# getzlab/rnaseqc

Hardware: AMD Instinct MI355X
Metric: reads/sec whole-node (100 M-read synthetic BAM, GENCODE GTF) at 1/2/4/8 GPU -- `value`: the hot path over the records resident in HBM (the bench contract's definition of value); `whole_node.value`: the same job from the BAM file to the reports (CLI `Average Reads/Sec` window), checked against `value (higher is better)
Workload: dtype i32/u64 counters, f64 exon fractions

## Files before the change

### rnaseqc_amd/csrc/rsqc_k1.h

```cpp
#pragma once

namespace rsqc {

#if defined(__HIP_DEVICE_COMPILE__)
#define K1E_LANDED(x) asm volatile("" : "+v"(x))
#ifdef K1E_PIN_ARGS
#define K1E_PIN(x) asm volatile("" : "+s"(x))
#else
#define K1E_PIN(x) (void)(x)
#endif
#else
#define K1E_LANDED(x) (void)(x)
#define K1E_PIN(x) (void)(x)
#endif

struct K1Args { DevAnnotation a; DevParams p; DevBatch b; DevAccum acc; };
#if defined(__HIPCC__)
__device__ __forceinline__ const K1Args *k1e_lazy_args() {
#if defined(__HIP_DEVICE_COMPILE__)
    const K1Args *q = (const K1Args *)__builtin_amdgcn_kernarg_segment_ptr();
    asm volatile("" : "+s"(q));
    return q;
#else
    return nullptr;
#endif
}
#else
static const K1Args *g_k1e_args = nullptr;
static unsigned long long g_k1e_coarse_hits = 0;
static unsigned long long g_k1e_ucache_hits = 0;
static unsigned long long g_k1e_uniform_calls = 0;
static unsigned long long g_k1e_uniform2_calls = 0;
static inline const K1Args *k1e_lazy_args() { return g_k1e_args; }
#endif

#ifndef K1E_NT
#define K1E_NT 0
#endif
template <class T> __device__ __forceinline__ T k1e_ld32_stream(const T *base, uint32_t idx) {
#if defined(__HIP_DEVICE_COMPILE__)
    if (K1E_NT & 1) {
        typedef uint32_t u32x4 __attribute__((ext_vector_type(4)));
        static_assert(sizeof(T) == 16, "16-byte streams");
        const u32x4 v = __builtin_nontemporal_load(reinterpret_cast<const u32x4 *>(reinterpret_cast<const char *>(base) + (uint32_t)(idx * 16u)));
        T r; __builtin_memcpy(&r, &v, 16); return r;
    }
#endif
    return ld32(base, idx);
}
struct alignas(4) Cig4 { uint32_t v[4]; };
__device__ __forceinline__ void k1e_load_cigar8(const uint32_t *cigar, uint32_t off, uint32_t (&c)[8]) {
    const char *const at = reinterpret_cast<const char *>(cigar) + (uint32_t)(off * 4u);
#if defined(__HIP_DEVICE_COMPILE__)
    if (K1E_NT & 1) {
        typedef uint32_t u32x4a __attribute__((ext_vector_type(4), aligned(4)));
        const u32x4a l4 = __builtin_nontemporal_load(reinterpret_cast<const u32x4a *>(at)), h4 = __builtin_nontemporal_load(reinterpret_cast<const u32x4a *>(at + 16));
        c[0] = l4.x; c[1] = l4.y; c[2] = l4.z; c[3] = l4.w; c[4] = h4.x; c[5] = h4.y; c[6] = h4.z; c[7] = h4.w;
        return;
    }
#endif
    const Cig4 lo = *reinterpret_cast<const Cig4 *>(at), hi = *reinterpret_cast<const Cig4 *>(at + 16);
#pragma unroll
    for (int k = 0; k < 4; ++k) { c[k] = lo.v[k]; c[4 + k] = hi.v[k]; }
}

#if defined(K1E_STOP_AT) && defined(__HIP_DEVICE_COMPILE__)
template <class T> __device__ __forceinline__ int k1e_keep_v(T x) { asm volatile("" :: "v"(x)); return 0; }
template <class T> __device__ __forceinline__ int k1e_keep_s(T x) { asm volatile("" :: "s"(x)); return 0; }
template <class... T> __device__ __forceinline__ void k1e_sink_v(T... x) { const int d[] = {k1e_keep_v(x)...}; (void)d; }
template <class... T> __device__ __forceinline__ void k1e_sink_s(T... x) { const int d[] = {k1e_keep_s(x)...}; (void)d; }
#define K1E_STOP(n, V, S) if (K1E_STOP_AT == (n)) { k1e_sink_v V; k1e_sink_s S; break; }
#else
#define K1E_STOP(n, V, S)
#endif
#if defined(K1E_STAGE_MARKS)
#define K1E_AMARK(sec)
#else
#define K1E_AMARK(sec) RSQC_MARK(sec)
#endif
constexpr int K1E_WAVES = RSQC_K1_THREADS / 64;
#ifndef K1E_PIECE_RECORDS
#define K1E_PIECE_RECORDS 256
#endif
constexpr uint64_t K1E_PIECE = K1E_PIECE_RECORDS;
#ifndef K1E_QCAP_N
#define K1E_QCAP_N 128
#endif
constexpr int K1E_QCAP = K1E_QCAP_N;
#ifndef K1E_ESLOTS_N
#define K1E_ESLOTS_N 256
#endif
#ifndef K1E_GSLOTS_N
#define K1E_GSLOTS_N 128
#endif
constexpr int K1E_ESLOTS = K1E_ESLOTS_N, K1E_GSLOTS = K1E_GSLOTS_N;
constexpr uint32_t K1E_HQ = 1u << 16;
#ifndef K1E_ABL
#define K1E_ABL 0
#endif
#ifndef K1E_WALK_SKIP
#define K1E_WALK_SKIP 1
#endif
#ifndef K1E_EXON_RUNSUM
#define K1E_EXON_RUNSUM 1
#endif

struct K1eTables {
    unsigned long long cnt[8];
    uint32_t cnt32[64];
    double eval[K1E_ESLOTS];
    uint32_t ekey[K1E_ESLOTS];
    unsigned long long gval[K1E_GSLOTS];
    uint32_t gkey[K1E_GSLOTS];
    uint32_t rl[3];
    uint32_t pairs;
    uint32_t frags;
    uint32_t piece;
    uint32_t defer;
    alignas(16) uint32_t ucache[K1E_WAVES][12];
    int32_t bedc[K1E_WAVES][4];
    static __device__ __forceinline__ constexpr int sum_slot(int c) {
        return c == RSQC_C_END1_MISMATCHES ? 0 : c == RSQC_C_END1_BASES ? 1 : c == RSQC_C_END2_MISMATCHES ? 2 : c == RSQC_C_END2_BASES ? 3 :
               c == RSQC_C_MISMATCHED_BASES ? 4 : c == RSQC_C_TOTAL_BASES ? 5 : c == RSQC_C_ALIGNMENT_BLOCKS ? 6 : 7;
    }
    __device__ __forceinline__ void init(uint32_t pairs0) {
        if (threadIdx.x < 8) cnt[threadIdx.x] = 0ull;
        if (threadIdx.x < 64) cnt32[threadIdx.x] = 0u;
        for (int c = threadIdx.x; c < K1E_ESLOTS; c += blockDim.x) { ekey[c] = 0xFFFFFFFFu; eval[c] = 0.0; }
        for (int c = threadIdx.x; c < K1E_GSLOTS; c += blockDim.x) { gkey[c] = 0xFFFFFFFFu; gval[c] = 0ull; }
        if (threadIdx.x == 0) { rl[0] = 0u; rl[1] = 0xFFFFFFFFu; rl[2] = 0u; pairs = pairs0; piece = 0u; frags = 0u; defer = 0u; }
        if (threadIdx.x < K1E_WAVES) { ucache[threadIdx.x][8] = 1u; ucache[threadIdx.x][9] = 0u; bedc[threadIdx.x][0] = -1; }
    }
    __device__ __forceinline__ void exon_add(uint32_t eid, double frac) {
        const uint32_t slot = eid & (K1E_ESLOTS - 1);
        const uint32_t old = atomicCAS(&ekey[slot], 0xFFFFFFFFu, eid);
        if (old == 0xFFFFFFFFu || old == eid) atomicAdd(&eval[slot], frac);
        else atomicAdd(&k1e_lazy_args()->acc.exon_acc[eid], frac);
    }
    __device__ __forceinline__ void gene_add(uint32_t g, uint32_t n, uint32_t nd) {
        const uint32_t slot = g & (K1E_GSLOTS - 1);
        const uint32_t old = atomicCAS(&gkey[slot], 0xFFFFFFFFu, g);
        if (old == 0xFFFFFFFFu || old == g) atomicAdd(&gval[slot], (unsigned long long)n | ((unsigned long long)nd << 32));
        else {
            const DevAccum &acc = k1e_lazy_args()->acc;
            atomicAdd(&acc.gene_reads[g], (unsigned long long)n); if (nd) atomicAdd(&acc.gene_unique[g], (unsigned long long)nd);
        }
    }
    __device__ __forceinline__ void flush(unsigned long long n_records) {
        const DevAccum &acc = k1e_lazy_args()->acc;
        for (int c = threadIdx.x; c < RSQC_N_COUNTERS; c += blockDim.x) {
            unsigned long long v = cnt[sum_slot(c)] + (unsigned long long)cnt32[c];
            if (c == RSQC_C_TOTAL_ALIGNMENTS) v += n_records;
            if (c == RSQC_C_MAPPED_UNIQUE_READS) v += (unsigned long long)cnt32[RSQC_C_MAPPED_READS] - cnt32[RSQC_C_MAPPED_DUPLICATE_READS];
            if (c == RSQC_C_UNIQUE_FRAGMENTS) v += (unsigned long long)cnt32[RSQC_C_END1_MAPPED_READS] - cnt32[RSQC_C_DUPLICATE_PAIRS];
            if (c == RSQC_C_LOW_QUALITY_READS) v += (unsigned long long)cnt32[RSQC_C_READS_USED] - cnt32[RSQC_C_HIGH_QUALITY_READS];
            if (v) atomicAdd(&acc.counters[c], v);
        }
        for (int c = threadIdx.x; c < K1E_ESLOTS; c += blockDim.x)
            if (ekey[c] != 0xFFFFFFFFu) atomicAdd(&acc.exon_acc[ekey[c]], eval[c]);
        for (int c = threadIdx.x; c < K1E_GSLOTS; c += blockDim.x)
            if (gkey[c] != 0xFFFFFFFFu) {
                const unsigned long long v = gval[c];
                atomicAdd(&acc.gene_reads[gkey[c]], v & 0xFFFFFFFFull);
                if (v >> 32) atomicAdd(&acc.gene_unique[gkey[c]], v >> 32);
            }
    }
};

struct K1eQueue1 { uint32_t bs[K1E_QCAP], lf[K1E_QCAP], idx[K1E_QCAP];
#ifdef K1E_COARSE
                   uint32_t cz[K1E_QCAP];
#endif
};
struct K1eQueue2 { uint32_t bs0[K1E_QCAP], len0[K1E_QCAP], bs1[K1E_QCAP], len1[K1E_QCAP], idx[K1E_QCAP], flhq[K1E_QCAP]; };
#ifndef K1E_Q3CAP_N
#define K1E_Q3CAP_N 84
#endif
constexpr int K1E_Q3CAP = K1E_Q3CAP_N;
static_assert(K1E_Q3CAP >= 64 && K1E_Q3CAP <= 128, "the three-block ring holds at least one full call");
struct K1eQueue3 { uint32_t bs0[K1E_Q3CAP], bs1[K1E_Q3CAP], bs2[K1E_Q3CAP], lens01[K1E_Q3CAP], lf2[K1E_Q3CAP], idx[K1E_Q3CAP]; };
__device__ __forceinline__ uint32_t k1e_wrap3(uint32_t s) { return s >= (uint32_t)K1E_Q3CAP ? s - (uint32_t)K1E_Q3CAP : s; }
struct K1eShared {
    K1eTables T;
    K1eQueue1 q1[K1E_WAVES];
    K1eQueue2 q2[K1E_WAVES];
    K1eQueue3 q3[K1E_WAVES];
#ifdef K1E_LDS_PAD
    char pad[K1E_LDS_PAD];
#endif
};

#if defined(__HIP_DEVICE_COMPILE__)
#define K1E_GLOBAL(T, p) ((__attribute__((address_space(1))) T *)(p))
#else
#define K1E_GLOBAL(T, p) (p)
#endif
struct K1ePairDst { uint64_t pairs; uint32_t cap; };
#ifndef K1E_LAZYPAIR
#define K1E_LAZYPAIR 1
#endif
__device__ __forceinline__ K1ePairDst k1e_pair_dst() {
    K1ePairDst d;
#if defined(__HIP_DEVICE_COMPILE__)
    const void *q = __builtin_amdgcn_kernarg_segment_ptr();
    asm volatile("s_load_dwordx2 %0, %2, %3\n\ts_load_dword %1, %2, %4\n\ts_waitcnt lgkmcnt(0)"
                 : "=&s"(d.pairs), "=&s"(d.cap)
                 : "s"(q), "n"(offsetof(K1Args, acc) + offsetof(DevAccum, pairs)), "n"(offsetof(K1Args, acc) + offsetof(DevAccum, pair_chunk_cap)));
#else
    const DevAccum &a = k1e_lazy_args()->acc;
    d.pairs = (uint64_t)(uintptr_t)a.pairs; d.cap = a.pair_chunk_cap;
#endif
    return d;
}
#ifndef K1E_CONSTMASK
#define K1E_CONSTMASK 1
#endif
__device__ __forceinline__ bool k1e_first_lane() { return K1E_CONSTMASK ? WaveSink::lane(LaneMask{1ull}) : lane_id() == 0; }
template <int N> __device__ __forceinline__ bool k1e_lane_below() { static_assert(N > 0 && N < 64, "lanes"); return K1E_CONSTMASK ? WaveSink::lane(LaneMask{(1ull << N) - 1ull}) : lane_id() < N; }

template <bool LANE_CHUNK = false>
__device__ __forceinline__ void k1e_emit_pairs(K1eTables &T, uint64_t m, uint32_t g, uint64_t qhash, uint32_t qh2, const K1ePairDst &pd, uint32_t chunk) {
    if (LANE_CHUNK) {
        if (WaveSink::lane(LaneMask{m})) {
            const uint32_t slot = atomicAdd(&k1e_lazy_args()->acc.pair_chunk_count[chunk], 1u);
            if (slot < pd.cap) K1E_GLOBAL(PairRec, (PairRec *)(uintptr_t)pd.pairs)[(size_t)chunk * pd.cap + slot] = PairRec{g, qh2, qhash};
            else atomicExch(k1e_lazy_args()->acc.error, RSQC_ERR_CAPACITY);
        }
        return;
    }
    const int lead = __ffsll((unsigned long long)m) - 1;
    uint32_t base = 0;
    if (lane_id() == lead) base = atomicAdd(&T.pairs, (uint32_t)__popcll(m));
    base = lane_value(base, lead);
    if (WaveSink::lane(LaneMask{m})) {
        const uint32_t slot = base + mask_rank(m);
        const size_t chunk_at = (size_t)chunk * pd.cap;
        if (slot < pd.cap) {
#if defined(__HIP_DEVICE_COMPILE__)
            if (K1E_NT & 2) {
                typedef uint32_t u32x4 __attribute__((ext_vector_type(4)));
                const u32x4 v = {g, qh2, (uint32_t)qhash, (uint32_t)(qhash >> 32)};
                __builtin_nontemporal_store(v, reinterpret_cast<u32x4 *>(K1E_GLOBAL(PairRec, (PairRec *)(uintptr_t)pd.pairs) + (chunk_at + slot)));
            } else
#endif
            K1E_GLOBAL(PairRec, (PairRec *)(uintptr_t)pd.pairs)[chunk_at + slot] = PairRec{g, qh2, qhash};
        } else atomicExch(k1e_lazy_args()->acc.error, RSQC_ERR_CAPACITY);
    }
}

template <int NB, bool LANE_CHUNK = false>
__device__ __forceinline__ void k1e_commit(uint32_t *cov_diff, K1eTables &T, const EiOut &eo, const uint32_t (&len)[NB], uint32_t fl,
                                           uint64_t qhash, uint32_t qh2, const K1ePairDst &held, uint32_t chunk) {
    typedef WaveSink WS;
    const K1ePairDst pd = K1E_LAZYPAIR ? k1e_pair_dst() : held;
    const uint64_t notdup = WS::prim((fl & RSQC_FDUP) == 0).m;
    double inv_aligned = 1.0;
    uint32_t aligned_of = 0; (void)aligned_of;
    if (NB > 1) {
        uint32_t aligned = 0;
#pragma unroll
        for (int b = 0; b < NB; ++b) aligned += len[b];
        inv_aligned = 1.0 / (double)(aligned ? aligned : 1u);
        aligned_of = aligned;
    }
#pragma unroll
    for (int k = 0; k < 2 * NB; ++k) {
        const uint64_t has = WS::prim(((eo.cmask >> k) & 1u) != 0).m;
        if (has == 0ull) continue;
        const uint32_t ln = len[k >> 1];
        const uint64_t hvm = has & WS::prim(ln > 0).m;
        const bool hv = WS::lane(LaneMask{hvm});
        if (NB == 1) {
            const RunLite r = make_run_lite(hvm, eo.eid[k]);
            if (r.head && !(K1E_ABL & 2)) T.exon_add(eo.eid[k], (double)r.count);
            if (k == 0) {
                const uint64_t nd = hvm & notdup;
                if (r.head && !(K1E_ABL & 2)) T.gene_add(eo.hit[0], r.count, run_popcount(nd, r.count));
            }
        } else if (!(K1E_ABL & 2)) {
#if K1E_EXON_RUNSUM
            const uint64_t cont = run_cont_mask(hvm, eo.eid[k]);
            if (cont == 0ull) { if (hv) T.exon_add(eo.eid[k], (double)ln * inv_aligned); }
            else {
                const uint32_t al = aligned_of;
                const uint64_t mixed_len = cont & WS::prim(lane_below(al) != al).m;
                if (mixed_len != 0ull) { if (hv) T.exon_add(eo.eid[k], (double)ln * inv_aligned); }
                else {
                    const uint32_t sc = wave_inclusive_scan_u32_dpp(hv ? ln : 0u);
                    const uint32_t cnt_run = run_length_at(cont);
                    const uint32_t at_end = lane_gather(sc, (uint32_t)lane_id() + cnt_run - 1u);
                    const bool head = WS::lane(LaneMask{hvm & ~cont});
                    if (head) T.exon_add(eo.eid[k], (double)(at_end - (sc - ln)) * inv_aligned);
                }
            }
#else
            if (hv) T.exon_add(eo.eid[k], (double)ln * inv_aligned);
#endif
        }
        const uint32_t base = hv ? eo.cidx[k] : 0u;
        if (!(K1E_ABL & 4)) {
            cov_add_merged(cov_diff, hvm, base, 1u);
            cov_add_merged(cov_diff, hvm, base + ln, 0xFFFFFFFFu);
        }
    }
#pragma unroll
    for (int k = 0; k < FAST_SET; ++k) {
        const uint64_t m = WS::prim(eo.n_hit > k).m;
        if (m == 0ull) break;
        const uint32_t g = eo.hit[k];
        if (!(K1E_ABL & 8)) k1e_emit_pairs<LANE_CHUNK>(T, m, g, qhash, qh2, pd, chunk);
        if (NB > 1 || k > 0) {
            const RunLite r = make_run_lite(m, g);
            const uint64_t nd = m & notdup;
            if (r.head && !(K1E_ABL & 2)) T.gene_add(g, r.count, run_popcount(nd, r.count));
        }
    }
}

constexpr uint64_t K1E_OVF_LONG = 1ull << 63;
constexpr uint32_t K1E_OVF_STAGE = 1024;
struct K1eStageCtl {
    uint32_t n;
    uint32_t end;
    __device__ __forceinline__ void init() { n = 0u; end = K1E_OVF_STAGE; }
    __device__ __forceinline__ uint32_t staged() const { return n < end ? n : end; }
};
__device__ __forceinline__ void k1e_overflow(bool over, uint64_t index, unsigned long long *stage = nullptr, K1eStageCtl *ctl = nullptr) {
    const uint64_t m = WaveSink::prim(over).m;
    if (m == 0ull) return;
    const int lead = __ffsll((unsigned long long)m) - 1;
    const uint32_t n = (uint32_t)__popcll(m);
    uint32_t base = 0;
    bool staged = false;
    if (stage) {
        if (lane_id() == lead) base = atomicAdd(&ctl->n, n);
        base = lane_value(base, lead);
        staged = base <= K1E_OVF_STAGE - n;
        if (staged && over) stage[base + mask_rank(m)] = index;
        if (!staged && lane_id() == lead) atomicMin(&ctl->end, base);
    }
    if (!staged) {
        const DevAccum &acc = k1e_lazy_args()->acc;
        if (lane_id() == lead) base = atomicAdd(acc.ovf_count, n);
        base = lane_value(base, lead);
        if (over) {
            const uint32_t slot = base + mask_rank(m);
            if (slot < acc.ovf_cap) acc.ovf_index[slot] = index;
            else atomicExch(acc.error, RSQC_ERR_CAPACITY);
        }
    }
}
__device__ __forceinline__ void k1e_stage_flush(const DevAccum &acc, const unsigned long long *stage, const K1eStageCtl *ctl, uint32_t *piece) {
    const uint32_t n_st = ctl->staged();
    if (n_st != 0u) {
        if (threadIdx.x == 0) *piece = atomicAdd(acc.ovf_count, n_st);
        __syncthreads();
        const uint32_t at = *piece;
        for (uint32_t j = threadIdx.x; j < n_st; j += blockDim.x) {
            if (at + j < acc.ovf_cap) acc.ovf_index[at + j] = stage[j];
            else atomicExch(acc.error, RSQC_ERR_CAPACITY);
        }
    }
}

#ifndef K1E_UNIFORM1
#define K1E_UNIFORM1 1
#endif
// ... 59 lines not shown
    if (p.stranded != RSQC_STRAND_UNKNOWN || ci.rk_words == 0u) return false;
    uint32_t *const uc = T.ucache[wave]; (void)uc;
    EiEntry S;
    bool cached = false;
#if K1E_UCACHE
    {
        const int32_t lo = (int32_t)__builtin_amdgcn_readfirstlane((int)uc[8]), hi = (int32_t)__builtin_amdgcn_readfirstlane((int)uc[9]);
        cached = (WS::prim(bs < lo || (int32_t)(bs + (int32_t)len) >= hi).m & onm) == 0ull;
        if (cached) {
            const uint4 e0 = *reinterpret_cast<const uint4 *>(uc), e1 = *reinterpret_cast<const uint4 *>(uc + 4);
#define K1E_U(x) ((uint32_t)__builtin_amdgcn_readfirstlane((int)(x)))
            S = EiEntry{(int32_t)K1E_U(e0.x), K1E_U(e0.y), K1E_U(e0.z), K1E_U(e0.w), K1E_U(e1.x), K1E_U(e1.y), K1E_U(e1.z), K1E_U(e1.w)};
#undef K1E_U
#if defined(RSQC_WAVE_EMU)
            if (lane_id() == 0) ++g_k1e_ucache_hits;
#endif
        }
    }
#endif
    if (!cached) {
        const K1eInterval iv = k1e_interval_of(a, ci, (int32_t)lane_value((uint32_t)bs, 0));
        S = iv.S;
        if (S.mask & EIM_DEEP) return false;
        const int32_t lo = S.pos, hi = iv.next_pos > S.pos ? iv.next_pos : 0x7FFFFFFF;
        if ((WS::prim(bs < lo || (int32_t)(bs + (int32_t)len) >= hi).m & onm) != 0ull) return false;
#if K1E_UCACHE
        if (k1e_first_lane()) {
            *reinterpret_cast<uint4 *>(uc) = make_uint4((uint32_t)S.pos, S.mask, S.eidA, S.eidB);
            *reinterpret_cast<uint4 *>(uc + 4) = make_uint4(S.gfA, S.cdA, S.gfB, S.cdB);
            *reinterpret_cast<uint2 *>(uc + 8) = make_uint2((uint32_t)lo, (uint32_t)hi);
        }
        k1e_wave_lds_visible();
#endif
    }
#if defined(RSQC_WAVE_EMU)
    if (lane_id() == 0) ++g_k1e_uniform_calls;
#endif
    const bool cA = S.eidA != EI_NONE, cB = S.eidB != EI_NONE, c1 = cA && cB;
    const uint32_t g0 = S.gfA & ROW_GENE_MASK, g1 = S.gfB & ROW_GENE_MASK;
    const uint32_t gX = cA ? g0 : g1, gfX = cA ? S.gfA : S.gfB;
    const bool va = cA || cB, vb = c1 && g1 != gX;
    const bool globin = (va && ((gfX >> ROW_FLAG_SHIFT) & ROWF_GLOBIN) != 0) || (vb && ((S.gfB >> ROW_FLAG_SHIFT) & ROWF_GLOBIN) != 0);
    const uint64_t hqm = WS::prim((flhq & K1E_HQ) != 0).m & onm, dupm = WS::prim((flhq & RSQC_FDUP) != 0).m;
    const uint32_t n_on = (uint32_t)__popcll(onm), n_hq = (uint32_t)__popcll(hqm);
    if (!globin) {
        RSQC_COUNT(cnt, RSQC_C_NON_GLOBIN_READS, LaneMask{onm}); RSQC_COUNT(cnt, RSQC_C_NON_GLOBIN_DUPLICATE_READS, LaneMask{onm & dupm});
    }
    k1e_uniform_class_counts(p, ei_class_flags(S.mask, RSQC_STRAND_UNKNOWN), va, flhq, onm, n_on, n_hq, cnt);
    if (!va || hqm == 0ull) return true;
    const uint64_t hvm = hqm & WS::prim(len > 0).m;
    if (hvm == 0ull) return true;
    const K1ePairDst pd = K1E_LAZYPAIR ? k1e_pair_dst() : held;
    const uint32_t n0 = (uint32_t)__popcll(hvm), nd0 = (uint32_t)__popcll(hvm & ~dupm);
    const bool first = k1e_first_lane();
    if (!(K1E_ABL & 2)) {
        if (first) { T.exon_add(cA ? S.eidA : S.eidB, (double)n0); T.gene_add(gX, n0, nd0); }
        if (first && c1) T.exon_add(S.eidB, (double)n0);
        if (first && vb) T.gene_add(g1, n0, nd0);
    }
    if (!(K1E_ABL & 4)) {
        const uint32_t base = (cA ? S.cdA : S.cdB) + (uint32_t)bs;
        cov_add_merged(cov_diff, hvm, base, 1u); cov_add_merged(cov_diff, hvm, base + len, 0xFFFFFFFFu);
        if (c1) { const uint32_t b1 = S.cdB + (uint32_t)bs; cov_add_merged(cov_diff, hvm, b1, 1u); cov_add_merged(cov_diff, hvm, b1 + len, 0xFFFFFFFFu); }
    }
    if (!(K1E_ABL & 8)) {
        k1e_emit_pairs(T, hvm, gX, qhash, qh2, pd, blockIdx.x);
        if (vb) k1e_emit_pairs(T, hvm, g1, qhash, qh2, pd, blockIdx.x);
    }
    return true;
}

#ifndef K1E_UNIFORM2
#define K1E_UNIFORM2 0
#endif
struct K1eInterval2 { EiEntry S[2]; int32_t next_pos[2]; uint32_t next_mask[2]; };
__device__ __forceinline__ K1eInterval2 k1e_intervals_of(const DevAnnotation &a, const ContigInfo &ci, int32_t x0, int32_t x1) {
    const int32_t top = (int32_t)(ci.rk_words << 6) - 1;
    const int32_t xc0 = x0 < 0 ? 0 : (x0 > top ? top : x0), xc1 = x1 < 0 ? 0 : (x1 > top ? top : x1);
    const uint32_t word0 = ci.rk_base + ((uint32_t)xc0 >> 6), word1 = ci.rk_base + ((uint32_t)xc1 >> 6);
    K1eInterval2 r;
#if defined(__HIP_DEVICE_COMPILE__)
    typedef uint32_t u32x4 __attribute__((ext_vector_type(4)));
    typedef uint32_t u32x16 __attribute__((ext_vector_type(16)));
    u32x4 w0, w1;
    asm volatile("s_load_dwordx4 %0, %2, %3\n\ts_load_dwordx4 %1, %2, %4\n\ts_waitcnt lgkmcnt(0)"
                 : "=&s"(w0), "=&s"(w1) : "s"(a.ei_rank), "s"(word0 * 16u), "s"(word1 * 16u));
    const uint64_t t0 = (((uint64_t)w0.y << 32) | (uint64_t)w0.x) << (63u - ((uint32_t)xc0 & 63u));
    const uint64_t t1 = (((uint64_t)w1.y << 32) | (uint64_t)w1.x) << (63u - ((uint32_t)xc1 & 63u));
    const uint32_t j0 = w0.z + (uint32_t)__popcll(t0) - 1u, j1 = w1.z + (uint32_t)__popcll(t1) - 1u;
    u32x16 e0, e1;
    asm volatile("s_load_dwordx16 %0, %2, %3\n\ts_load_dwordx16 %1, %2, %4\n\ts_waitcnt lgkmcnt(0)"
                 : "=&s"(e0), "=&s"(e1) : "s"(a.ei), "s"(j0 * 32u), "s"(j1 * 32u));
    r.S[0] = EiEntry{(int32_t)e0.s0, e0.s1, e0.s2, e0.s3, e0.s4, e0.s5, e0.s6, e0.s7}; r.next_pos[0] = (int32_t)e0.s8; r.next_mask[0] = e0.s9;
    r.S[1] = EiEntry{(int32_t)e1.s0, e1.s1, e1.s2, e1.s3, e1.s4, e1.s5, e1.s6, e1.s7}; r.next_pos[1] = (int32_t)e1.s8; r.next_mask[1] = e1.s9;
#else
    const int32_t xc[2] = {xc0, xc1}; const uint32_t word[2] = {word0, word1};
    for (int b = 0; b < 2; ++b) {
        const EiRank w = a.ei_rank[word[b]];
        const uint64_t t = (((uint64_t)w.hi << 32) | (uint64_t)w.lo) << (63u - ((uint32_t)xc[b] & 63u));
        const uint32_t j = w.rank + (uint32_t)__builtin_popcountll(t) - 1u;
        r.S[b] = a.ei[j]; r.next_pos[b] = a.ei[j + 1].pos; r.next_mask[b] = a.ei[j + 1].mask;
    }
#endif
    return r;
}
__device__ __forceinline__ bool k1e_uniform2(const DevAnnotation &a, const DevParams &p, uint32_t *cov_diff, const ContigInfo &ci, K1eTables &T,
                                             const int32_t (&bs)[2], const uint32_t (&len)[2], uint32_t flhq, uint64_t qhash, uint32_t qh2,
                                             uint64_t onm, WaveSink &cnt, const K1ePairDst &held) {
    typedef WaveSink WS;
    if (p.stranded != RSQC_STRAND_UNKNOWN || ci.rk_words == 0u) return false;
    const K1eInterval2 iv = k1e_intervals_of(a, ci, (int32_t)lane_value((uint32_t)bs[0], 0), (int32_t)lane_value((uint32_t)bs[1], 0));
    if ((iv.S[0].mask | iv.S[1].mask) & EIM_DEEP) return false;
    uint32_t mask = 0;
#pragma unroll
    for (int b = 0; b < 2; ++b) {
        const int32_t lo = iv.S[b].pos, hi = iv.next_pos[b] > iv.S[b].pos ? iv.next_pos[b] : 0x7FFFFFFF;
        const int32_t be = bs[b] + (int32_t)len[b];
        if ((WS::prim(bs[b] < lo || bs[b] >= hi || be > hi).m & onm) != 0ull) return false;
        const uint64_t touch = WS::prim(be == hi).m & onm;
        if (touch != 0ull && touch != onm) return false;
        mask |= iv.S[b].mask | (touch != 0ull ? iv.next_mask[b] & ~EIM_DEEP : 0u);
    }
#if defined(RSQC_WAVE_EMU)
    if (lane_id() == 0) ++g_k1e_uniform2_calls;
#endif
    uint32_t eid[4], cd[4], con = 0, ma = 0, mb = 0, la = 0, lb = 0;
    bool va = false, vb = false, ga = false, gb = false;
#pragma unroll
    for (int b = 0; b < 2; ++b) {
        const EiEntry &S = iv.S[b];
        const bool cA = S.eidA != EI_NONE, cB = S.eidB != EI_NONE, c0 = cA || cB, c1 = cA && cB;
        const uint32_t g0 = S.gfA & ROW_GENE_MASK, g1 = S.gfB & ROW_GENE_MASK;
        const uint32_t gX = cA ? g0 : g1, gfX = cA ? S.gfA : S.gfB;
        eid[2 * b] = cA ? S.eidA : S.eidB; cd[2 * b] = cA ? S.cdA : S.cdB; eid[2 * b + 1] = S.eidB; cd[2 * b + 1] = S.cdB;
        con |= (c0 ? 1u : 0u) << (2 * b) | (c1 ? 1u : 0u) << (2 * b + 1);
        if (b == 0) {
            la = gX; va = c0; ga = c0 && ((gfX >> ROW_FLAG_SHIFT) & ROWF_GLOBIN) != 0;
            lb = g1; vb = c1 && g1 != gX; gb = vb && ((S.gfB >> ROW_FLAG_SHIFT) & ROWF_GLOBIN) != 0;
            ma = (c0 ? 1u : 0u) | ((c1 && g1 == gX) ? 2u : 0u); mb = vb ? 2u : 0u;
        } else {
            const bool a_in = (c0 && la == gX) || (c1 && la == g1), b_in = (c0 && lb == gX) || (c1 && lb == g1);
            va = va && a_in; vb = vb && b_in;
            ma |= ((c0 && la == gX) ? 1u : 0u) << 2 | ((c1 && la == g1) ? 1u : 0u) << 3;
            mb |= ((c0 && lb == gX) ? 1u : 0u) << 2 | ((c1 && lb == g1) ? 1u : 0u) << 3;
        }
    }
    ga = ga && va; gb = gb && vb;
    const bool any_gene = va || vb;
    const uint64_t hqm = WS::prim((flhq & K1E_HQ) != 0).m & onm, dupm = WS::prim((flhq & RSQC_FDUP) != 0).m;
    const uint32_t n_on = (uint32_t)__popcll(onm), n_hq = (uint32_t)__popcll(hqm);
    if (!(ga || gb)) {
        RSQC_COUNT(cnt, RSQC_C_NON_GLOBIN_READS, LaneMask{onm}); RSQC_COUNT(cnt, RSQC_C_NON_GLOBIN_DUPLICATE_READS, LaneMask{onm & dupm});
    }
    k1e_uniform_class_counts(p, ei_class_flags(mask, RSQC_STRAND_UNKNOWN), any_gene, flhq, onm, n_on, n_hq, cnt);
    if (!any_gene || hqm == 0ull) return true;
    const uint32_t cmask = con & ((va ? ma : 0u) | (vb ? mb : 0u));
    const K1ePairDst pd = K1E_LAZYPAIR ? k1e_pair_dst() : held;
    const uint32_t aligned = len[0] + len[1];
    const bool first = k1e_first_lane();
#pragma unroll
    for (int b = 0; b < 2; ++b) {
        const uint32_t bits = (cmask >> (2 * b)) & 3u;
        if (bits == 0u) continue;
        const uint32_t ln = len[b];
        const uint64_t hvm = hqm & WS::prim(ln > 0).m;
        if (hvm == 0ull) continue;
        const bool hv = WS::lane(LaneMask{hvm});
        if (!(K1E_ABL & 2)) {
            const uint32_t al0 = lane_value(aligned, __ffsll((unsigned long long)hvm) - 1);
            if ((hvm & WS::prim(aligned != al0).m) == 0ull) {
                const uint32_t tot = wave_sum_u32_full(hv ? ln : 0u);
                const double frac = (double)tot * (1.0 / (double)al0);
                if (first && (bits & 1u)) T.exon_add(eid[2 * b], frac);
                if (first && (bits & 2u)) T.exon_add(eid[2 * b + 1], frac);
            } else if (hv) {
                const double frac = (double)ln * (1.0 / (double)aligned);
                if (bits & 1u) T.exon_add(eid[2 * b], frac);
                if (bits & 2u) T.exon_add(eid[2 * b + 1], frac);
            }
        }
        if (!(K1E_ABL & 4)) {
#pragma unroll
            for (int j = 0; j < 2; ++j)
                if (bits & (1u << j)) {
                    const uint32_t base = cd[2 * b + j] + (uint32_t)bs[b];
                    cov_add_merged(cov_diff, hvm, base, 1u); cov_add_merged(cov_diff, hvm, base + ln, 0xFFFFFFFFu);
                }
        }
    }
    const uint64_t m = hqm & WS::prim(aligned > 0).m;
    if (m == 0ull) return true;
    const uint32_t n0 = (uint32_t)__popcll(m), nd0 = (uint32_t)__popcll(m & ~dupm);
    const uint32_t hit0 = va ? la : lb;
    if (!(K1E_ABL & 8)) k1e_emit_pairs(T, m, hit0, qhash, qh2, pd, blockIdx.x);
    if (first && !(K1E_ABL & 2)) T.gene_add(hit0, n0, nd0);
    if (va && vb) {
        if (!(K1E_ABL & 8)) k1e_emit_pairs(T, m, lb, qhash, qh2, pd, blockIdx.x);
        if (first && !(K1E_ABL & 2)) T.gene_add(lb, n0, nd0);
    }
    return true;
}

constexpr uint32_t K1E_TAB_BLOCK3 = CIG_BLOCK_SET | (CIG_BLOCK_SET << 16), K1E_TAB_REF3 = CIG_REF_SET | (CIG_REF_SET << 16), K1E_TAB_BAD3 = 0xFE00FE00u;
template <int NB>
__device__ __forceinline__ void k1e_process(const DevAnnotation &a, const DevParams &p, const rsqc_rec_aux *aux, uint32_t *cov_diff,
                                            const ContigInfo &ci, K1eShared &S, int wave, uint32_t head, uint32_t n,
                                            const uint32_t *qh2col, const K1ePairDst &held) {
    static_assert(NB >= 1 && NB <= 3, "queues of one-, two- and three-block records");
    const int l = lane_id();
    const bool on = (uint32_t)l < n;
    const uint32_t slot = NB == 3 ? k1e_wrap3(head + (uint32_t)l) : ((head + (uint32_t)l) & (K1E_QCAP - 1));
    int32_t bs[NB]; uint32_t len[NB]; uint32_t idx, flhq, pre0 = 0u;
    if (NB == 1) {
        const K1eQueue1 &q = S.q1[wave];
        const uint32_t lf = q.lf[slot];
        bs[0] = (int32_t)q.bs[slot]; len[0] = lf & 0xFFFFu; idx = q.idx[slot];
#ifdef K1E_COARSE
        pre0 = q.cz[slot];
#endif
        flhq = ((lf >> 16) & 0xFFFu) | ((lf >> 28) << 16);
    } else if (NB == 2) {
        const K1eQueue2 &q = S.q2[wave];
        bs[0] = (int32_t)q.bs0[slot]; len[0] = q.len0[slot]; bs[NB - 1] = (int32_t)q.bs1[slot]; len[NB - 1] = q.len1[slot]; idx = q.idx[slot]; flhq = q.flhq[slot];
    } else {
        const K1eQueue3 &q = S.q3[wave];
        const uint32_t l01 = q.lens01[slot], lf = q.lf2[slot];
        bs[0] = (int32_t)q.bs0[slot]; len[0] = l01 & 0xFFFFu; bs[NB > 1 ? 1 : 0] = (int32_t)q.bs1[slot]; len[NB > 1 ? 1 : 0] = l01 >> 16;
        bs[NB - 1] = (int32_t)q.bs2[slot]; len[NB - 1] = lf & 0xFFFFu; idx = q.idx[slot];
        flhq = ((lf >> 16) & 0xFFFu) | ((lf >> 28) << 16);
    }
    if (!on) { idx = 0u; flhq = 0u; pre0 = 0u; }
#if defined(RSQC_WAVE_EMU)
    if (pre0) ++g_k1e_coarse_hits;
#endif
    const uint2 qh = ld32(reinterpret_cast<const uint2 *>(aux), idx * 2u);
    const uint32_t qh2 = qh2col ? ld32(qh2col, idx) : 0u;
    K1E_SMARK(1);
    WaveSink cnt;
    const uint64_t onm = n >= 64u ? ~0ull : (1ull << n) - 1ull;
    bool done = false;
    if (NB == 1 && K1E_UNIFORM1) done = k1e_uniform1(a, p, cov_diff, ci, S.T, bs[0], len[0], flhq, (uint64_t)qh.x | ((uint64_t)qh.y << 32), qh2, onm, cnt, held, wave);
    if (NB == 2 && K1E_UNIFORM2) {
        const int32_t b2[2] = {bs[0], bs[NB - 1]}; const uint32_t l2[2] = {len[0], len[NB - 1]};
        done = k1e_uniform2(a, p, cov_diff, ci, S.T, b2, l2, flhq, (uint64_t)qh.x | ((uint64_t)qh.y << 32), qh2, onm, cnt, held);
    }
    if (!done) {
        EiOut eo; bool over = false;
        exon_metrics_ei<NB, WaveSink>(a, p, ci, flhq & 0xFFFFu, bs, len, (flhq & K1E_HQ) != 0, eo, over, cnt, on, (uint32_t)NB, pre0);
        k1e_overflow(on && over, (uint64_t)idx);
        k1e_commit<NB>(cov_diff, S.T, eo, len, flhq, (uint64_t)qh.x | ((uint64_t)qh.y << 32), qh2, held, blockIdx.x);
        K1E_SMARK(6);
// ... 550 lines not shown
```

### rnaseqc_amd/csrc/rsqc_wave.h

```cpp
#pragma once

namespace rsqc {

__device__ __forceinline__ int lane_id() { return (int)(threadIdx.x & 63u); }

__device__ __forceinline__ uint32_t lane_below(uint32_t v) {
#if defined(__HIP_DEVICE_COMPILE__)
    return (uint32_t)__builtin_amdgcn_update_dpp((int)v, (int)v, 0x138, 0xf, 0xf, false);
#else
    return __shfl_up(v, 1, 64);
#endif
}

__device__ __forceinline__ uint32_t bfe_u(uint32_t src, uint32_t off, uint32_t width) {
#if defined(__HIP_DEVICE_COMPILE__)
    return __builtin_amdgcn_ubfe(src, off, width);
#else
    return (src >> (off & 31u)) & ((width & 31u) ? ((1u << (width & 31u)) - 1u) : 0u);
#endif
}
__device__ __forceinline__ uint32_t bfe_m(uint32_t src, uint32_t off) {
#if defined(__HIP_DEVICE_COMPILE__)
    return (uint32_t)__builtin_amdgcn_sbfe((int)src, off, 1u);
#else
// ... 73 lines not shown
    return v;
}

__device__ __forceinline__ uint32_t wave_inclusive_scan_u32_dpp(uint32_t v) {
#if defined(__HIP_DEVICE_COMPILE__)
#define RSQC_DPP_SCAN(ctrl, rmask) { v += (uint32_t)__builtin_amdgcn_update_dpp(0, (int)v, ctrl, rmask, 0xf, false); }
    RSQC_DPP_SCAN(0x111, 0xf) RSQC_DPP_SCAN(0x112, 0xf) RSQC_DPP_SCAN(0x114, 0xf) RSQC_DPP_SCAN(0x118, 0xf)
    RSQC_DPP_SCAN(0x142, 0xa) RSQC_DPP_SCAN(0x143, 0xc)
#undef RSQC_DPP_SCAN
    return v;
#else
    return wave_inclusive_scan_u32(v);
#endif
}
__device__ __forceinline__ uint32_t lane_gather(uint32_t v, uint32_t src) {
#if defined(__HIP_DEVICE_COMPILE__)
    return (uint32_t)__builtin_amdgcn_ds_bpermute((int)((src & 63u) << 2), (int)v);
#else
    return __shfl(v, (int)(src & 63u), 64);
#endif
}

template <class F>
__device__ __forceinline__ void wave_aggregate(bool valid, uint32_t key, uint64_t flagmask, F &&leader) {
    uint64_t todo = __ballot(valid);
    const int l = lane_id();
    while (todo) {
        const int lead = __ffsll((unsigned long long)todo) - 1;
        const uint32_t k0 = __shfl(key, lead, 64);
        const uint64_t same = __ballot(valid && key == k0);
        if (l == lead) leader(k0, (uint32_t)__popcll(same), (uint32_t)__popcll(same & flagmask));
        todo &= ~same;
    }
}

struct Run { bool head; uint32_t count; int end; uint64_t mask; };
__device__ __forceinline__ Run make_run(uint64_t vmask, uint32_t key) {
    const int l = lane_id();
    const uint32_t pk = lane_below(key);
    const uint64_t neq = WaveSink::prim(pk != key).m;
    const uint64_t headm = vmask & (~(vmask << 1) | neq);
    Run r;
    r.head = WaveSink::lane(LaneMask{headm});
    const uint64_t stop = headm | ~vmask;
    const uint64_t above = l == 63 ? 0ull : stop & ~((2ull << l) - 1ull);
    r.end = above ? __ffsll((unsigned long long)above) - 1 : 64;
    r.count = (uint32_t)(r.end - l);
    const uint64_t upto = r.end == 64 ? ~0ull : ((1ull << r.end) - 1ull);
    r.mask = upto & ~((1ull << l) - 1ull);
    return r;
}
__device__ __forceinline__ Run make_run(bool valid, uint32_t key) { return make_run(WaveSink::prim(valid).m, key); }

struct RunLite { bool head; uint32_t count; };
__device__ __forceinline__ uint64_t run_cont_mask(uint64_t vmask, uint32_t key) {
    const uint32_t pk = lane_below(key);
    return vmask & (vmask << 1) & ~WaveSink::prim(pk != key).m;
}
__device__ __forceinline__ uint32_t run_length_at(uint64_t cont) {
    const uint64_t t = (cont >> 1) >> (uint32_t)lane_id();
    const uint32_t lo = ~(uint32_t)t, hi = ~(uint32_t)(t >> 32);
#if defined(__HIP_DEVICE_COMPILE__)
    uint32_t a, fh;
    asm("v_ffbl_b32 %0, %1" : "=v"(a) : "v"(lo));
    asm("v_ffbl_b32 %0, %1" : "=v"(fh) : "v"(hi));
    const uint32_t b2 = 32u + fh;
#else
    const uint32_t a = lo ? (uint32_t)__builtin_ctz(lo) : 0xFFFFFFFFu, b2 = 32u + (hi ? (uint32_t)__builtin_ctz(hi) : 0xFFFFFFFFu);
#endif
    return 1u + (a < b2 ? a : b2);
}
__device__ __forceinline__ RunLite make_run_lite(uint64_t vmask, uint32_t key) {
    const uint64_t cont = run_cont_mask(vmask, key);
    RunLite r;
    r.head = WaveSink::lane(LaneMask{vmask & ~cont});
    r.count = run_length_at(cont);
    return r;
}
__device__ __forceinline__ uint32_t run_popcount(uint64_t m, uint32_t count) {
    const uint64_t t = m >> (uint32_t)lane_id();
    const uint64_t keep = count >= 64u ? ~0ull : ((1ull << count) - 1ull);
    return (uint32_t)__popcll(t & keep);
}
__device__ __forceinline__ double run_sum_f64(double v, const Run &r) {
    const int l = lane_id();
    double sc = v;
#pragma unroll
    for (int o = 1; o < 64; o <<= 1) { const double t = __shfl_up(sc, o, 64); if (l >= o) sc += t; }
    const double at_end = __shfl(sc, r.end - 1, 64);
    return at_end - (sc - v);
}

__device__ __forceinline__ uint32_t run_sum_u32(uint32_t v, const Run &r) {
    const uint32_t sc = wave_inclusive_scan_u32(v);
    const uint32_t at_end = __shfl(sc, r.end - 1, 64);
    return at_end - (sc - v);
}

#ifndef RSQC_COV_MERGE_MIN
#define RSQC_COV_MERGE_MIN 1
#endif
__device__ __forceinline__ void cov_add_merged(uint32_t *cov, uint64_t vmask, uint32_t idx, uint32_t sign) {
    const uint64_t cont = run_cont_mask(vmask, idx);
    if (__popcll(cont) < RSQC_COV_MERGE_MIN) {
        if (WaveSink::lane(LaneMask{vmask})) atomicAdd(&cov[idx], sign);
    } else {
        const uint32_t n = run_length_at(cont);
        if (WaveSink::lane(LaneMask{vmask & ~cont})) atomicAdd(&cov[idx], sign * n);
    }
}
__device__ __forceinline__ void cov_add_merged(uint32_t *cov, bool valid, uint32_t idx, uint32_t sign) {
    cov_add_merged(cov, WaveSink::prim(valid).m, idx, sign);
}

__device__ __forceinline__ uint32_t find_segment(const DevBatch &b, uint64_t i) {
    uint32_t lo = 0, hi = b.n_seg;
    while (hi - lo > 1) { const uint32_t m = (lo + hi) >> 1; if (b.seg_start[m] <= i) lo = m; else hi = m; }
    return lo;
}


}
```

Baseline: 26.46 billion.

## Move shared-table spill paths to cold noinline helpers and share coverage run masks

Exon and gene accumulation into the LDS hash tables now take a wave lane mask. Lanes that collide in the table are gathered into a ballot mask and handed to noinline cold helpers that do the global atomics, and a new combined exon_gene_add issues both CAS operations together. Coverage diff updates compute run heads for the start and end offsets once, relative to the block, and reuse them across the two exon copies. The pair-capacity error path is also moved out of line. The aim is to cut divergent branches, register pressure and repeated run-mask work in the hot loop, at the cost of extra ballots and a function call when misses occur.

New measurement: 26.40 billion. No clear change (-0.2%).

```diff
diff --git a/rnaseqc_amd/csrc/rsqc_k1.h b/rnaseqc_amd/csrc/rsqc_k1.h
--- a/rnaseqc_amd/csrc/rsqc_k1.h
+++ b/rnaseqc_amd/csrc/rsqc_k1.h
@@ -31,8 +31,31 @@
 static unsigned long long g_k1e_ucache_hits = 0;
 static unsigned long long g_k1e_uniform_calls = 0;
 static unsigned long long g_k1e_uniform2_calls = 0;
+static unsigned long long g_k1e_cold_lanes[3] = {0, 0, 0};
 static inline const K1Args *k1e_lazy_args() { return g_k1e_args; }
 #endif
+
+static __device__ __attribute__((noinline, cold)) void k1e_exon_to_memory(const K1Args *q, uint64_t miss, uint32_t eid, double frac) {
+#if defined(RSQC_WAVE_EMU)
+    if (lane_id() == 0) g_k1e_cold_lanes[0] += (unsigned long long)__builtin_popcountll(miss);
+#endif
+    if (WaveSink::lane(LaneMask{miss})) atomicAdd(&q->acc.exon_acc[eid], frac);
+}
+static __device__ __attribute__((noinline, cold)) void k1e_gene_to_memory(const K1Args *q, uint64_t miss, uint32_t g, uint32_t n, uint32_t nd) {
+#if defined(RSQC_WAVE_EMU)
+    if (lane_id() == 0) g_k1e_cold_lanes[1] += (unsigned long long)__builtin_popcountll(miss);
+#endif
+    if (WaveSink::lane(LaneMask{miss})) {
+        const DevAccum &acc = q->acc;
+        atomicAdd(&acc.gene_reads[g], (unsigned long long)n); if (nd) atomicAdd(&acc.gene_unique[g], (unsigned long long)nd);
+    }
+}
+static __device__ __attribute__((noinline, cold)) void k1e_capacity_error(const K1Args *q) {
+#if defined(RSQC_WAVE_EMU)
+    if (lane_id() == 0) ++g_k1e_cold_lanes[2];
+#endif
+    if (lane_id() == 0) atomicExch(q->acc.error, RSQC_ERR_CAPACITY);
+}
 
 #ifndef K1E_NT
 #define K1E_NT 0
@@ -131,20 +154,38 @@
         if (threadIdx.x == 0) { rl[0] = 0u; rl[1] = 0xFFFFFFFFu; rl[2] = 0u; pairs = pairs0; piece = 0u; frags = 0u; defer = 0u; }
         if (threadIdx.x < K1E_WAVES) { ucache[threadIdx.x][8] = 1u; ucache[threadIdx.x][9] = 0u; bedc[threadIdx.x][0] = -1; }
     }
-    __device__ __forceinline__ void exon_add(uint32_t eid, double frac) {
-        const uint32_t slot = eid & (K1E_ESLOTS - 1);
-        const uint32_t old = atomicCAS(&ekey[slot], 0xFFFFFFFFu, eid);
-        if (old == 0xFFFFFFFFu || old == eid) atomicAdd(&eval[slot], frac);
-        else atomicAdd(&k1e_lazy_args()->acc.exon_acc[eid], frac);
-    }
-    __device__ __forceinline__ void gene_add(uint32_t g, uint32_t n, uint32_t nd) {
-        const uint32_t slot = g & (K1E_GSLOTS - 1);
-        const uint32_t old = atomicCAS(&gkey[slot], 0xFFFFFFFFu, g);
-        if (old == 0xFFFFFFFFu || old == g) atomicAdd(&gval[slot], (unsigned long long)n | ((unsigned long long)nd << 32));
-        else {
-            const DevAccum &acc = k1e_lazy_args()->acc;
-            atomicAdd(&acc.gene_reads[g], (unsigned long long)n); if (nd) atomicAdd(&acc.gene_unique[g], (unsigned long long)nd);
-        }
+    static __device__ __forceinline__ bool taken(uint32_t old, uint32_t key) { return old != 0xFFFFFFFFu && old != key; }
+    __device__ __forceinline__ void exon_add(uint64_t m, uint32_t eid, double frac) {
+        bool miss = false;
+        if (WaveSink::lane(LaneMask{m})) {
+            const uint32_t slot = eid & (K1E_ESLOTS - 1);
+            miss = taken(atomicCAS(&ekey[slot], 0xFFFFFFFFu, eid), eid);
+            atomicAdd(&eval[slot], miss ? 0.0 : frac);
+        }
+        const uint64_t mm = WaveSink::prim(miss).m;
+        if (mm != 0ull) k1e_exon_to_memory(k1e_lazy_args(), mm, eid, frac);
+    }
+    __device__ __forceinline__ void gene_add(uint64_t m, uint32_t g, uint32_t n, uint32_t nd) {
+        bool miss = false;
+        if (WaveSink::lane(LaneMask{m})) {
+            const uint32_t slot = g & (K1E_GSLOTS - 1);
+            miss = taken(atomicCAS(&gkey[slot], 0xFFFFFFFFu, g), g);
+            atomicAdd(&gval[slot], miss ? 0ull : (unsigned long long)n | ((unsigned long long)nd << 32));
+        }
+        const uint64_t mm = WaveSink::prim(miss).m;
+        if (mm != 0ull) k1e_gene_to_memory(k1e_lazy_args(), mm, g, n, nd);
+    }
+    __device__ __forceinline__ void exon_gene_add(uint64_t m, uint32_t eid, double frac, uint32_t g, uint32_t n, uint32_t nd) {
+        bool emiss = false, gmiss = false;
+        if (WaveSink::lane(LaneMask{m})) {
+            const uint32_t es = eid & (K1E_ESLOTS - 1), gs = g & (K1E_GSLOTS - 1);
+            const uint32_t eold = atomicCAS(&ekey[es], 0xFFFFFFFFu, eid), gold = atomicCAS(&gkey[gs], 0xFFFFFFFFu, g);
+            emiss = taken(eold, eid); gmiss = taken(gold, g);
+            atomicAdd(&eval[es], emiss ? 0.0 : frac);
+            atomicAdd(&gval[gs], gmiss ? 0ull : (unsigned long long)n | ((unsigned long long)nd << 32));
+        }
+        const uint64_t em = WaveSink::prim(emiss).m, gm = WaveSink::prim(gmiss).m;
+        if ((em | gm) != 0ull) { const K1Args *q = k1e_lazy_args(); k1e_exon_to_memory(q, em, eid, frac); k1e_gene_to_memory(q, gm, g, n, nd); }
     }
     __device__ __forceinline__ void flush(unsigned long long n_records) {
         const DevAccum &acc = k1e_lazy_args()->acc;
@@ -221,31 +262,33 @@
 template <bool LANE_CHUNK = false>
 __device__ __forceinline__ void k1e_emit_pairs(K1eTables &T, uint64_t m, uint32_t g, uint64_t qhash, uint32_t qh2, const K1ePairDst &pd, uint32_t chunk) {
     if (LANE_CHUNK) {
+        bool over = false;
         if (WaveSink::lane(LaneMask{m})) {
             const uint32_t slot = atomicAdd(&k1e_lazy_args()->acc.pair_chunk_count[chunk], 1u);
-            if (slot < pd.cap) K1E_GLOBAL(PairRec, (PairRec *)(uintptr_t)pd.pairs)[(size_t)chunk * pd.cap + slot] = PairRec{g, qh2, qhash};
-            else atomicExch(k1e_lazy_args()->acc.error, RSQC_ERR_CAPACITY);
-        }
+            over = slot >= pd.cap;
+            if (!over) K1E_GLOBAL(PairRec, (PairRec *)(uintptr_t)pd.pairs)[(size_t)chunk * pd.cap + slot] = PairRec{g, qh2, qhash};
+        }
+        if (WaveSink::prim(over).m != 0ull) k1e_capacity_error(k1e_lazy_args());
         return;
     }
     const int lead = __ffsll((unsigned long long)m) - 1;
     uint32_t base = 0;
-    if (lane_id() == lead) base = atomicAdd(&T.pairs, (uint32_t)__popcll(m));
+    if (WaveSink::lane(LaneMask{m & (0ull - m)})) base = atomicAdd(&T.pairs, (uint32_t)__popcll(m));
     base = lane_value(base, lead);
-    if (WaveSink::lane(LaneMask{m})) {
-        const uint32_t slot = base + mask_rank(m);
+    const uint32_t slot = base + mask_rank(m);
+    const uint64_t fit = m & WaveSink::prim(slot < pd.cap).m;
+    if (WaveSink::lane(LaneMask{fit})) {
         const size_t chunk_at = (size_t)chunk * pd.cap;
-        if (slot < pd.cap) {
 #if defined(__HIP_DEVICE_COMPILE__)
-            if (K1E_NT & 2) {
-                typedef uint32_t u32x4 __attribute__((ext_vector_type(4)));
-                const u32x4 v = {g, qh2, (uint32_t)qhash, (uint32_t)(qhash >> 32)};
-                __builtin_nontemporal_store(v, reinterpret_cast<u32x4 *>(K1E_GLOBAL(PairRec, (PairRec *)(uintptr_t)pd.pairs) + (chunk_at + slot)));
-            } else
-#endif
-            K1E_GLOBAL(PairRec, (PairRec *)(uintptr_t)pd.pairs)[chunk_at + slot] = PairRec{g, qh2, qhash};
-        } else atomicExch(k1e_lazy_args()->acc.error, RSQC_ERR_CAPACITY);
-    }
+        if (K1E_NT & 2) {
+            typedef uint32_t u32x4 __attribute__((ext_vector_type(4)));
+            const u32x4 v = {g, qh2, (uint32_t)qhash, (uint32_t)(qhash >> 32)};
+            __builtin_nontemporal_store(v, reinterpret_cast<u32x4 *>(K1E_GLOBAL(PairRec, (PairRec *)(uintptr_t)pd.pairs) + (chunk_at + slot)));
+        } else
+#endif
+        K1E_GLOBAL(PairRec, (PairRec *)(uintptr_t)pd.pairs)[chunk_at + slot] = PairRec{g, qh2, qhash};
+    }
+    if (fit != m) k1e_capacity_error(k1e_lazy_args());
 }
 
 template <int NB, bool LANE_CHUNK = false>
@@ -271,36 +314,32 @@
         const uint64_t hvm = has & WS::prim(ln > 0).m;
         const bool hv = WS::lane(LaneMask{hvm});
         if (NB == 1) {
-            const RunLite r = make_run_lite(hvm, eo.eid[k]);
-            if (r.head && !(K1E_ABL & 2)) T.exon_add(eo.eid[k], (double)r.count);
-            if (k == 0) {
-                const uint64_t nd = hvm & notdup;
-                if (r.head && !(K1E_ABL & 2)) T.gene_add(eo.hit[0], r.count, run_popcount(nd, r.count));
-            }
+            const RunHeads r = make_run_heads(hvm, eo.eid[k]);
+            if (K1E_ABL & 2) {}
+            else if (k == 0) T.exon_gene_add(r.head, eo.eid[k], (double)r.count, eo.hit[0], r.count, run_popcount(hvm & notdup, r.count));
+            else T.exon_add(r.head, eo.eid[k], (double)r.count);
         } else if (!(K1E_ABL & 2)) {
+            uint64_t am = hvm;
+            double val = (double)ln * inv_aligned;
 #if K1E_EXON_RUNSUM
             const uint64_t cont = run_cont_mask(hvm, eo.eid[k]);
-            if (cont == 0ull) { if (hv) T.exon_add(eo.eid[k], (double)ln * inv_aligned); }
-            else {
+            if (cont != 0ull) {
                 const uint32_t al = aligned_of;
                 const uint64_t mixed_len = cont & WS::prim(lane_below(al) != al).m;
-                if (mixed_len != 0ull) { if (hv) T.exon_add(eo.eid[k], (double)ln * inv_aligned); }
-                else {
+                if (mixed_len == 0ull) {
                     const uint32_t sc = wave_inclusive_scan_u32_dpp(hv ? ln : 0u);
                     const uint32_t cnt_run = run_length_at(cont);
                     const uint32_t at_end = lane_gather(sc, (uint32_t)lane_id() + cnt_run - 1u);
-                    const bool head = WS::lane(LaneMask{hvm & ~cont});
-                    if (head) T.exon_add(eo.eid[k], (double)(at_end - (sc - ln)) * inv_aligned);
+                    am = hvm & ~cont;
+                    val = (double)(at_end - (sc - ln)) * inv_aligned;
                 }
             }
-#else
-            if (hv) T.exon_add(eo.eid[k], (double)ln * inv_aligned);
-#endif
-        }
-        const uint32_t base = hv ? eo.cidx[k] : 0u;
+#endif
+            T.exon_add(am, eo.eid[k], val);
+        }
         if (!(K1E_ABL & 4)) {
-            cov_add_merged(cov_diff, hvm, base, 1u);
-            cov_add_merged(cov_diff, hvm, base + ln, 0xFFFFFFFFu);
+            const uint32_t base = hv ? eo.cidx[k] : 0u;
+            cov_add_block(cov_diff, make_cov_runs(hvm, base, ln), base, ln);
         }
     }
 #pragma unroll
@@ -309,10 +348,9 @@
         if (m == 0ull) break;
         const uint32_t g = eo.hit[k];
         if (!(K1E_ABL & 8)) k1e_emit_pairs<LANE_CHUNK>(T, m, g, qhash, qh2, pd, chunk);
-        if (NB > 1 || k > 0) {
-            const RunLite r = make_run_lite(m, g);
-            const uint64_t nd = m & notdup;
-            if (r.head && !(K1E_ABL & 2)) T.gene_add(g, r.count, run_popcount(nd, r.count));
+        if ((NB > 1 || k > 0) && !(K1E_ABL & 2)) {
+            const RunHeads r = make_run_heads(m, g);
+            T.gene_add(r.head, g, r.count, run_popcount(m & notdup, r.count));
         }
     }
 }
@@ -478,16 +516,15 @@
     if (hvm == 0ull) return true;
     const K1ePairDst pd = K1E_LAZYPAIR ? k1e_pair_dst() : held;
     const uint32_t n0 = (uint32_t)__popcll(hvm), nd0 = (uint32_t)__popcll(hvm & ~dupm);
-    const bool first = k1e_first_lane();
     if (!(K1E_ABL & 2)) {
-        if (first) { T.exon_add(cA ? S.eidA : S.eidB, (double)n0); T.gene_add(gX, n0, nd0); }
-        if (first && c1) T.exon_add(S.eidB, (double)n0);
-        if (first && vb) T.gene_add(g1, n0, nd0);
+        T.exon_gene_add(1ull, cA ? S.eidA : S.eidB, (double)n0, gX, n0, nd0);
+        if (c1) T.exon_add(1ull, S.eidB, (double)n0);
+        if (vb) T.gene_add(1ull, g1, n0, nd0);
     }
     if (!(K1E_ABL & 4)) {
-        const uint32_t base = (cA ? S.cdA : S.cdB) + (uint32_t)bs;
-        cov_add_merged(cov_diff, hvm, base, 1u); cov_add_merged(cov_diff, hvm, base + len, 0xFFFFFFFFu);
-        if (c1) { const uint32_t b1 = S.cdB + (uint32_t)bs; cov_add_merged(cov_diff, hvm, b1, 1u); cov_add_merged(cov_diff, hvm, b1 + len, 0xFFFFFFFFu); }
+        const CovRuns runs = make_cov_runs(hvm, (uint32_t)bs, len);
+        cov_add_block(cov_diff, runs, (cA ? S.cdA : S.cdB) + (uint32_t)bs, len);
+        if (c1) cov_add_block(cov_diff, runs, S.cdB + (uint32_t)bs, len);
     }
     if (!(K1E_ABL & 8)) {
         k1e_emit_pairs(T, hvm, gX, qhash, qh2, pd, blockIdx.x);
@@ -583,7 +620,6 @@
     const uint32_t cmask = con & ((va ? ma : 0u) | (vb ? mb : 0u));
     const K1ePairDst pd = K1E_LAZYPAIR ? k1e_pair_dst() : held;
     const uint32_t aligned = len[0] + len[1];
-    const bool first = k1e_first_lane();
 #pragma unroll
     for (int b = 0; b < 2; ++b) {
         const uint32_t bits = (cmask >> (2 * b)) & 3u;
@@ -597,21 +633,19 @@
             if ((hvm & WS::prim(aligned != al0).m) == 0ull) {
                 const uint32_t tot = wave_sum_u32_full(hv ? ln : 0u);
                 const double frac = (double)tot * (1.0 / (double)al0);
-                if (first && (bits & 1u)) T.exon_add(eid[2 * b], frac);
-                if (first && (bits & 2u)) T.exon_add(eid[2 * b + 1], frac);
-            } else if (hv) {
+                if (bits & 1u) T.exon_add(1ull, eid[2 * b], frac);
+                if (bits & 2u) T.exon_add(1ull, eid[2 * b + 1], frac);
+            } else {
                 const double frac = (double)ln * (1.0 / (double)aligned);
-                if (bits & 1u) T.exon_add(eid[2 * b], frac);
-                if (bits & 2u) T.exon_add(eid[2 * b + 1], frac);
+                if (bits & 1u) T.exon_add(hvm, eid[2 * b], frac);
+                if (bits & 2u) T.exon_add(hvm, eid[2 * b + 1], frac);
             }
         }
         if (!(K1E_ABL & 4)) {
+            const CovRuns runs = make_cov_runs(hvm, (uint32_t)bs[b], ln);
 #pragma unroll
             for (int j = 0; j < 2; ++j)
-                if (bits & (1u << j)) {
-                    const uint32_t base = cd[2 * b + j] + (uint32_t)bs[b];
-                    cov_add_merged(cov_diff, hvm, base, 1u); cov_add_merged(cov_diff, hvm, base + ln, 0xFFFFFFFFu);
-                }
+                if (bits & (1u << j)) cov_add_block(cov_diff, runs, cd[2 * b + j] + (uint32_t)bs[b], ln);
         }
     }
     const uint64_t m = hqm & WS::prim(aligned > 0).m;
@@ -619,10 +653,10 @@
     const uint32_t n0 = (uint32_t)__popcll(m), nd0 = (uint32_t)__popcll(m & ~dupm);
     const uint32_t hit0 = va ? la : lb;
     if (!(K1E_ABL & 8)) k1e_emit_pairs(T, m, hit0, qhash, qh2, pd, blockIdx.x);
-    if (first && !(K1E_ABL & 2)) T.gene_add(hit0, n0, nd0);
+    if (!(K1E_ABL & 2)) T.gene_add(1ull, hit0, n0, nd0);
     if (va && vb) {
         if (!(K1E_ABL & 8)) k1e_emit_pairs(T, m, lb, qhash, qh2, pd, blockIdx.x);
-        if (first && !(K1E_ABL & 2)) T.gene_add(lb, n0, nd0);
+        if (!(K1E_ABL & 2)) T.gene_add(1ull, lb, n0, nd0);
     }
     return true;
 }
diff --git a/rnaseqc_amd/csrc/rsqc_wave.h b/rnaseqc_amd/csrc/rsqc_wave.h
--- a/rnaseqc_amd/csrc/rsqc_wave.h
+++ b/rnaseqc_amd/csrc/rsqc_wave.h
@@ -149,7 +149,6 @@
 }
 __device__ __forceinline__ Run make_run(bool valid, uint32_t key) { return make_run(WaveSink::prim(valid).m, key); }
 
-struct RunLite { bool head; uint32_t count; };
 __device__ __forceinline__ uint64_t run_cont_mask(uint64_t vmask, uint32_t key) {
     const uint32_t pk = lane_below(key);
     return vmask & (vmask << 1) & ~WaveSink::prim(pk != key).m;
@@ -167,13 +166,6 @@
 #endif
     return 1u + (a < b2 ? a : b2);
 }
-__device__ __forceinline__ RunLite make_run_lite(uint64_t vmask, uint32_t key) {
-    const uint64_t cont = run_cont_mask(vmask, key);
-    RunLite r;
-    r.head = WaveSink::lane(LaneMask{vmask & ~cont});
-    r.count = run_length_at(cont);
-    return r;
-}
 __device__ __forceinline__ uint32_t run_popcount(uint64_t m, uint32_t count) {
     const uint64_t t = m >> (uint32_t)lane_id();
     const uint64_t keep = count >= 64u ? ~0ull : ((1ull << count) - 1ull);
@@ -194,20 +186,40 @@
     return at_end - (sc - v);
 }
 
-#ifndef RSQC_COV_MERGE_MIN
-#define RSQC_COV_MERGE_MIN 1
-#endif
+struct RunHeads { uint64_t head; uint32_t count; };
+__device__ __forceinline__ RunHeads make_run_heads(uint64_t vmask, uint32_t key) {
+    const uint64_t cont = run_cont_mask(vmask, key);
+    RunHeads r;
+    r.head = vmask & ~cont;
+    r.count = 1u;
+    if (cont != 0ull) r.count = run_length_at(cont);
+    return r;
+}
 __device__ __forceinline__ void cov_add_merged(uint32_t *cov, uint64_t vmask, uint32_t idx, uint32_t sign) {
-    const uint64_t cont = run_cont_mask(vmask, idx);
-    if (__popcll(cont) < RSQC_COV_MERGE_MIN) {
-        if (WaveSink::lane(LaneMask{vmask})) atomicAdd(&cov[idx], sign);
-    } else {
-        const uint32_t n = run_length_at(cont);
-        if (WaveSink::lane(LaneMask{vmask & ~cont})) atomicAdd(&cov[idx], sign * n);
-    }
+    const RunHeads r = make_run_heads(vmask, idx);
+    if (WaveSink::lane(LaneMask{r.head})) atomicAdd(&cov[idx], sign * r.count);
 }
 __device__ __forceinline__ void cov_add_merged(uint32_t *cov, bool valid, uint32_t idx, uint32_t sign) {
     cov_add_merged(cov, WaveSink::prim(valid).m, idx, sign);
+}
+struct CovRuns { uint64_t head_a, head_b; uint32_t n_a, n_b; };
+__device__ __forceinline__ CovRuns make_cov_runs(uint64_t vmask, uint32_t rel, uint32_t ln) {
+    const uint64_t cont_a = run_cont_mask(vmask, rel), cont_b = run_cont_mask(vmask, rel + ln);
+    CovRuns r;
+    r.head_a = vmask & ~cont_a; r.head_b = vmask & ~cont_b;
+    r.n_a = 1u;
+    if (cont_a != 0ull) r.n_a = run_length_at(cont_a);
+    r.n_b = r.n_a;
+    if (cont_b != cont_a) r.n_b = cont_b != 0ull ? run_length_at(cont_b) : 1u;
+    return r;
+}
+__device__ __forceinline__ void cov_add_block(uint32_t *cov, const CovRuns &r, uint32_t base, uint32_t ln) {
+    if (r.head_a == r.head_b) {
+        if (WaveSink::lane(LaneMask{r.head_a})) { atomicAdd(&cov[base], r.n_a); atomicAdd(&cov[base + ln], 0u - r.n_a); }
+    } else {
+        if (WaveSink::lane(LaneMask{r.head_a})) atomicAdd(&cov[base], r.n_a);
+        if (WaveSink::lane(LaneMask{r.head_b})) atomicAdd(&cov[base + ln], 0u - r.n_b);
+    }
 }
 
 __device__ __forceinline__ uint32_t find_segment(const DevBatch &b, uint64_t i) {
```
